# ghostshell202/FluidFramework

Measured on AMD Instinct MI355X. Metric: sequenced ops applied/sec (whole node) over 100k docs, bit-exact summaries, higher is better.
Workload: dtype int32

## Files before the change

### fluidframework_amd/csrc/apply.hip.h

```cpp
#pragma once
#include <hip/hip_runtime.h>
#include <stdint.h>

#include <type_traits>

#include "../../include/mtr_synth.h"
#include "../../include/mtr_types.h"

#define MTR_DI __device__ __forceinline__
#ifndef MTR_COLD_NOINLINE
#define MTR_COLD_NOINLINE 0
#endif
#if MTR_COLD_NOINLINE
#define MTR_COLD __device__ __attribute__((noinline))
#else
#define MTR_COLD MTR_DI
#endif
#ifndef MTR_UNSWITCH
#define MTR_UNSWITCH 1
#endif

namespace mtr {

constexpr int NT = 64;
// ... 122 lines not shown
    uint32_t* heap;
    uint16_t* text;
    uint32_t* prop;
    uint32_t* rm;
    int32_t segcap, hcap, tcap, pcap, rcap;
    int32_t rtab;
    int32_t cap;
    int32_t lhcap;
    int32_t global_mode;
    uint32_t* scratch;
    int32_t ops_this_launch;
    int32_t new_length_calc;
    uint32_t n_docs;
    const uint32_t* doc_list;
    uint32_t n_launch;
    const mtr_op* ops;
    const mtr_doc_desc* docs;
    const uint16_t* btext;
    const uint32_t* propop_off;
    const uint32_t* propop_kv;
    const uint32_t* key_index;
    const uint32_t* val_eq;
    unsigned long long* stat_ops;
    uint32_t* delta;
    const uint64_t* doff;
    const uint32_t* dkind;
    const uint32_t* dpart;
    int32_t gen;
    int32_t gen_grow;
    mtr_synth_cfg gen_cfg;
    mtr_synth_state* gen_state;
    mtr_op* gen_ops;
    uint16_t* gen_text;
    unsigned long long* prof;
    uint32_t* pend;
    int32_t* csum;
    int32_t* umap;
    uint32_t* refs;
    int32_t refcap;
};

enum { P_OP = 0, P_PREFIX, P_SPLIT, P_SHIFT, P_INSERT, P_RANGE, P_ZAMBONI, P_ZBLOCK, P_COMPACT, P_FINDUID,
       P_TEXTGC, P_LOADSTORE, P_TEXTCOPY, P_UPDSEQ, P_NZBLOCK, P_NCOMPACT, P_SCOUR1, P_PACK, P_NLQ, P_PMATCH,
       P_TAPPEND, P_HEAP, P_OVERFLOW, P_NPACK, P_NMERGE, P_NPMATCH, P_NNLQ, P_SPLIT1, P_INS1, P_FETCH, P_X1, P_X2,
       P_PFSUM, P_PFDIRTY, P_MAT, P_CSUM, P_NCH, P_NLISTED, P_NDIRTY,
       P_SPREAD, P_CHUNKOF, P_NSPREAD,
       P_LOAD, P_PRE, P_VIEW, P_POST,
       P_NSUP, P_NDCH,
       P_HELPER,
       P_SINK,
       P_OVB, P_OVPB, P_NOVFB, P_NOVL,
       P_SUPREF, P_PXLIST, P_PXEVAL, P_PXSYNC, P_NPXR,
       P_NWALK, P_NDRND, P_WALK,
       P_COUNT };

enum { CP_TEXT = 0, CP_PROP, CP_RM, CP_RT, CP_DELTA, CP_POFF, CP_PKV, CP_KIX, CP_VEQ, CP_HDR, CP_PEND, CP_CSUM, CP_UMAP,
       CP_REFS, CP_N };

struct Sc {
    unsigned long long cp[CP_N];
    int gen_ref, gen_client;
    int rel[2];
    int relmask;
    int nrefs, refcap;
    int fail_op, max_heap, heap_need;
    int sepoch;
    int vref;
    unsigned long long sum_s, sum_l;
#ifdef MTR_PROF
    unsigned long long prof[P_COUNT];
#endif
};

struct St {
    int nseg, height, minseq, curseq;
    int collab, local, heapn, uidnext;
    int textused, propused, rmused, status;
    int texthalf;
    int htop;
    int dused;
    int holes;
    int chunked;
    int cur_op;
};

struct View {
    int ref;
    uint32_t client;
    int local;
};

template <bool G>
struct Doc {
    template <class T>
    using A = typename std::conditional<G, gptr<T>, lptr<T>>::type;
    A<int> len, seq, rseq, E, hseq;
    A<uint32_t> meta, text, props, uid, huid;
    lptr<Sc> sc;
    lptr<mtr_synth_state> gst;
    lptr<int> sx;
    int dcap;
    int cap, lhcap, rtmask;
    MTR_DI unsigned long long cold(int k) const {
        const unsigned long long v = sc->cp[k];
        return (unsigned long long)(uint32_t)__builtin_amdgcn_readfirstlane(int(uint32_t(v))) |
               ((unsigned long long)(uint32_t)__builtin_amdgcn_readfirstlane(int(uint32_t(v >> 32))) << 32);
    }
// ... 246 lines not shown
                         (newlen ? vp_lt(minseq, rseq) : vis);
        int inr = first;
        if (__ballot(walk != 0)) {
#ifdef MTR_PROF
            PROF_COUNT(P_NWALK);
            ProfScope _prof_walk(L.sc, P_WALK);
#endif
            const int iw = slotp ? (walk != 0 ? *slotp : 0) : i;
            inr |= -later_remover(L, iw, walk != 0, v.client);
        }
        if (newlen) {
            const int live = vis & len;
            const int gone = live & ~(~after | inr);
            return vp_sel(rem, vp_le(rseq, minseq) | gone, live);
        }
        const int seen = len & ~(rem & inr);
        const int r = vp_sel(vis, seen, rem & (X ? vp_lt(rseq, LOCAL_BASE) : -1));
        return r | (rem & ~after);
    }
    static MTR_DI int later_remover(const D& L, int i, bool walk, uint32_t c) {
        int inr = 0;
        if (walk) {
            uint32_t cell = rm_get(L, L.uid[i]);
            while (cell != 0xffffffu) {
                const uint32_t w = L.grm()[cell];
                if ((w >> 24) == c) {
                    inr = 1;
                    break;
                }
                cell = w & 0xffffffu;
            }
        }
        return inr;
    }

    static MTR_DI int local_length(const D& L, const St& s) {
        int sum = 0;
        for (int base = 0; base < s.nseg; base += 64) {
            const int i = base + lane_id();
            int x = 0;
            if (i < s.nseg && L.rseq[i] == RNONE) x = L.len[i];
            sum += rdlane(wave_incl_scan(x), 63);
        }
        return sum;
    }

    static constexpr int EMASK = 0x7fffffff;
    static MTR_DI int ev(int e, int eprev) { return e < 0 ? -1 : e - (eprev & EMASK); }
#ifndef MTR_GK
#define MTR_GK 4
#endif
    static constexpr int GK = MTR_GK;

    static MTR_DI void prefix(D& L, const St& s, const View& v, int newlen) {
        PROF(P_PREFIX);
        const int S = s.nseg;
        const int ln = lane_id();
        int carry = 0;
        if constexpr (G) {
            for (int base = 0; base < S; base += 64 * GK) {
                Hot hk[GK];
#pragma unroll
                for (int q = 0; q < GK; q++) hk[q] = ld_hot(L, min(base + 64 * q + ln, S - 1));
#pragma unroll
                for (int q = 0; q < GK; q++) {
                    if (base + 64 * q >= S) break;
                    const int i = base + 64 * q + ln;
                    const int x0 = vis_hot(L, hk[q], i, v, newlen, s.minseq, i < S);
                    const int in = vp_lt(i, S);
                    const int x = x0 & in;
                    const int inc = wave_incl_scan(max(x, 0));
                    L.E[vp_sel(in, i, S)] = (carry + inc) | (x & int(0x80000000u));
                    carry += rdlane(inc, 63);
                }
            }
            wsync();
            return;
        }
        if (MTR_UNSWITCH && !v.local && !newlen) prefix_lds<0, 0>(L, s, v, 0);
        else prefix_lds<-1, -1>(L, s, v, newlen);
        wsync();
    }
    template <int LOC, int NL>
    static MTR_DI void prefix_lds(D& L, const St& s, const View& v, int newlen) {
        const int S = s.nseg;
        const int ln = lane_id();
        int carry = 0;
        Hot h = S > 0 ? ld_hot(L, ln) : Hot{};
        for (int base = 0; base < S; base += 64) {
            const int i = base + ln;
            const Hot cur = h;
            if (base + 64 < S) h = ld_hot(L, i + 64);
            const int x0 = vis_hot<LOC, NL>(L, cur, i, v, newlen, s.minseq, i < S);
            const int in = vp_lt(i, S);
            const int x = x0 & in;
            const int inc = wave_incl_scan(max(x, 0));
            L.E[vp_sel(in, i, S)] = (carry + inc) | (x & int(0x80000000u));
            carry += rdlane(inc, 63);
        }
    }

    static MTR_DI int nsup(const D& L) { return sup_rows(L.cap); }
    static MTR_DI int nchr(const D& L) { return L.cap / 64 + 1; }
    static MTR_DI gptr<int> cs_rec(const D& L, int c) { return L.gcsum() + c * kCsumRows; }
    static MTR_DI gptr<int> cs_sl(const D& L) { return L.gcsum() + kCsumRows * nchr(L); }
    static MTR_DI gptr<int> cs_se(const D& L) { return cs_sl(L) + nsup(L); }
    static MTR_DI lptr<int> sup_pre(const D& L) { return L.sx; }
    static MTR_DI lptr<int> sup_fill(const D& L) { return L.sx + nsup(L); }
    static MTR_DI lptr<int> sup_mark(const D& L) { return L.sx + 2 * nsup(L); }
    static MTR_DI lptr<int> sup_len(const D& L) { return L.sx + 3 * nsup(L); }
    static MTR_DI lptr<int> sup_ev(const D& L) { return L.sx + 4 * nsup(L); }
    static MTR_DI lptr<int> sup_dlen(const D& L) { return L.sx + 5 * nsup(L); }
    static MTR_DI lptr<int> dlist(const D& L) { return L.sx + 6 * nsup(L); }
    static MTR_DI lptr<int> ch_ev(const D& L) { return dlist(L) + kListCap; }
    static MTR_DI lptr<int> ch_x(const D& L) { return ch_ev(L) + nchr(L); }
    static MTR_DI v4i ld4(gptr<const int> p) { return *(gptr<const v4i>)p; }
    static MTR_DI void csum_update(D& L, const St& s, int lo, int hi) {
        PROF(P_CSUM);
        if constexpr (G) {
            if (!s.chunked) return;
            hi = min(hi, s.nseg);
            if (lo >= hi) return;
            const int c0 = max(lo, 0) >> 6, c1 = (hi - 1) >> 6;
            for (int cb = c0; cb <= c1; cb += GK) {
                uint32_t mq[GK];
                int lq[GK], sqq[GK], rq[GK];
#pragma unroll
                for (int g = 0; g < GK; g++) {
                    const int ic = min((cb + g) * 64 + lane_id(), s.nseg - 1);
                    mq[g] = L.meta[ic];
                    lq[g] = L.len[ic];
                    sqq[g] = L.seq[ic];
                    rq[g] = L.rseq[ic];
                }
#pragma unroll
                for (int g = 0; g < GK; g++) {
                    const int c = cb + g;
                    if (c > c1) break;
                    const int i = c * 64 + lane_id();
                    const bool in = i < s.nseg;
                    const uint32_t m = mq[g];
                    const int len = lq[g], sq = sqq[g], rs = rq[g];
                    const bool live = in && !(m & M_DEL);
                    const bool rem = rs != RNONE;
                    const bool win = live && (sq > s.minseq || (rem && rs > s.minseq));
                    const uint64_t wm = __ballot(win);
                    const int nw = __popcll(wm);
                    int x = (live && !rem) ? len : 0;
                    int fx = (live && !rem && !win) ? len : 0;
                    int ev = live ? max(sq, rem ? rs : 0) : 0;
                    x = rdlane(wave_incl_scan(x), 63);
                    fx = rdlane(wave_incl_scan(fx), 63);
// ... 423 lines not shown
        const int x = ch_ev(L)[cc] > vref ? ch_x(L)[cc] : cl;
        const int inc = wave_incl_scan(c < nch ? x : 0);
        if (c < nch) ch_x(L)[c] = inc;
        if (lane_id() == 0) sup_fill(L)[q] = ep;
        wsync();
        return inc;
    }
    static MTR_DI void materialize(D& L, const St& s, const View& v, int newlen, int c0, int c1) {
        PROF(P_MAT);
        const int S = s.nseg, ln = lane_id();
        const lptr<int> spre = sup_pre(L);
        int qcur = -1, rel = 0;
        for (int cb = c0; cb <= c1; cb += GK) {
            Hot h[GK];
#pragma unroll
            for (int k = 0; k < GK; k++) h[k] = ld_hot(L, min(min(cb + k, c1) * 64 + ln, S - 1));
#pragma unroll
            for (int k = 0; k < GK; k++) {
                const int c = cb + k;
                if (c > c1) break;
                const int q = c >> 6;
                if (q != qcur && (c & 63)) {
                    rel = sup_row(L, s, q);
                    qcur = q;
                }
                const int base = (q > 0 ? uni(spre[q - 1]) : 0) + ((c & 63) ? rdlane(rel, (c & 63) - 1) : 0);
                const int i = c * 64 + ln;
                const int x0 = vis_hot(L, h[k], i, v, newlen, s.minseq, i < S);
                const int x = i < S ? x0 : 0;
                const int inc = wave_incl_scan(max(x, 0));
                if (i < S) L.E[i] = (base + inc) | (x < 0 ? int(0x80000000u) : 0);
            }
        }
        wsync();
    }
    static MTR_DI int chunk_of(D& L, const St& s, int nch, int pos) {
        PROF(P_CHUNKOF);
        const int ns = (nch + 63) >> 6, ln = lane_id();
        const lptr<int> spre = sup_pre(L);
        int q = -1;
        for (int b = 0; b < ns; b += 64) {
            const uint64_t m = __ballot(b + ln < ns && spre[min(b + ln, ns - 1)] >= pos);
            if (m) {
                q = b + first_lane(m);
                break;
            }
        }
        if (q < 0) return nch - 1;
        const int rel = sup_row(L, s, q);
        const int base = q > 0 ? uni(spre[q - 1]) : 0;
        const uint64_t m = __ballot(q * 64 + ln < nch && base + rel >= pos);
        return m ? q * 64 + first_lane(m) : nch - 1;
    }
    static MTR_DI int view_scan(D& L, St& s, const View& v, int newlen, int p_lo, int p_hi, bool bounded = false) {
        PROF(P_VIEW);
        if constexpr (G) {
            L.rhi = 0;
            if (s.chunked && s.nseg > 0) {
                const int total = prefix2(L, s, v, newlen, bounded ? p_hi + 1 : INT32_MAX);
                const int nch = (s.nseg + 63) >> 6;
                const int c0 = max(0, chunk_of(L, s, nch, p_lo) - 1);
                const int c1 = min(nch - 1, chunk_of(L, s, nch, p_hi + 1) + 2);
                materialize(L, s, v, newlen, c0, c1);
                L.rlo = c0 * 64;
                L.rhi = (c1 + 1) * 64;
                return total;
            }
        }
        prefix(L, s, v, newlen);
        return s.nseg > 0 ? (uni(L.E[s.nseg - 1]) & EMASK) : 0;
    }

    static MTR_DI void find1(const D& L, const St& s, const View& v, int pos, int& i_out, int& before, int newlen) {
        const int S = s.nseg;
        const int ln = lane_id();
        int c = 0;
        i_out = S;
        before = 0;
        for (int base = 0; base < S; base += 64) {
            const int i = base + ln;
            const Hot h = ld_hot(L, min(i, S - 1));
            const int x0 = vis_hot(L, h, i, v, newlen, s.minseq, i < S);
            const int x = (i < S) ? max(x0, 0) : 0;
            const int inc = wave_incl_scan(x);
            const uint64_t m = __ballot((i < S) & (c + inc > pos));
            if (m) {
                const int l = first_lane(m);
                i_out = base + l;
                before = c + rdlane(inc - x, l);
                return;
            }
            c += rdlane(inc, 63);
        }
        before = c;
    }

    static MTR_DI void containing(char* smem, const KParams& P, uint32_t d, int pos, int ref, int client, int32_t* out) {
        D L;
        carve(L, smem, P, d);
        St s;
        load_doc(L, P, s, d);
        View v;
        v.ref = ref;
        v.client = enc_client(client);
        v.local = (!s.collab || uint32_t(s.local) == v.client) ? 1 : 0;
        int i, before;
        find1(L, s, v, pos, i, before, P.new_length_calc);
        const int li = (G && s.holes && i < s.nseg) ? count_live(L, 0, i) : i;
        if (lane_id() == 0) {
            if (i >= s.nseg || pos < 0) {
                out[0] = -1;
                out[9] = before;
            } else {
                const uint32_t m = L.meta[i];
                out[0] = li;
                out[1] = pos - before;
                out[2] = L.len[i];
                out[3] = L.seq[i];
                out[4] = dec_client(m & M_CLIENT_MASK);
                out[5] = L.rseq[i] == RNONE ? -1 : L.rseq[i];
                out[6] = (m & M_MARKER) ? 1 : 0;
                out[7] = int(L.text[i]);
// ... 2419 lines not shown
#pragma unroll
            for (int q = 0; q < ZK; q++) {
                const int i = wb + 64 * q + ln;
                const bool it = i < hi && !(mq[q] & M_DEL) && (l == 2 || bnd_of(mq[q]) >= l - 2);
                const uint64_t mask = __ballot(it);
                const int k = n + __popcll(mask & lanes_below());
                if (it && k < 64) lst[k] = i;
                n += __popcll(mask);
            }
        }
        int T = n, off = 0;
        if (W > 1) {
            const lptr<int> row = tbox(L) + 16;
            if (ln == 0) row[w] = n;
            __syncthreads();
            T = 0;
            for (int u = 0; u < W; u++) {
                const int nu = uni(row[u]);
                if (u < w) off += nu;
                T += nu;
                if (nu > 64) T = -(1 << 20);
            }
        } else if (n > 64) {
            T = -1;
        }
        if (T < 0) return -1;
        if (T == 0) return 0;
        const int c = max(1, min(kMaxNodesInBlock - 1, T / (kMaxNodesInBlock / 2)));
        const int base = T / c;
        const int rem = T % c;
        const int big = rem * (base + 1);
        wsync();
        if (ln < n) {
            const int i = lst[ln];
            uint32_t m = L.meta[i];
            const int item = off + ln;
            const bool isStart = item < big ? item % (base + 1) == 0 : (item - big) % base == 0;
            const int nb = item == 0 ? top : (isStart ? l - 1 : (l == 2 ? 0 : l - 2));
            m = set_bnd(m, nb);
            if (l == 2 && isStart) m = set_ns(m, NS_UNDEF);
            L.meta[i] = m;
        }
        wsync();
        return c;
    }

    static MTR_DI int zamboni_block(D& L, const KParams& P, St& s, int x, int& to) {
        PROF(P_ZBLOCK);
        PROF_COUNT(P_NZBLOCK);
        const int H = s.height;
        int rs1, re1;
        block_bounds1(L, s, x, rs1, re1);
        const uint32_t m1 = uniu(L.meta[rs1]);
        if (ns_of(m1) == NS_FALSE) return -1;
        const int topb1 = bnd_of(m1);
        const int before = G && s.holes ? count_live(L, rs1, re1) : re1 - rs1;
        to = re1;
        int kept;
        {
            PROF(P_SCOUR1);
            kept = re1 - rs1 <= 64 ? scour_par(L, P, s, rs1, re1) : scour_gather(L, P, s, rs1, re1);
            if (kept < 0) kept = scour_range(L, P, s, rs1, re1);
        }
        for (int b = rs1; b < re1; b += 64) {
            const int i = b + lane_id();
            const uint64_t m = __ballot(i < re1 && !(L.meta[min(i, re1 - 1)] & M_DEL));
            if (m) {
                const int first = b + first_lane(m);
                L.meta[first] = set_ns(set_bnd(uniu(L.meta[first]), topb1), NS_FALSE);
                wsync();
                break;
            }
        }
        if (kept >= before) return -1;
        int from = rs1;
        if (kept < kMaxNodesInBlock / 2 && H > 1) {
            PROF(P_PACK);
            PROF_COUNT(P_NPACK);
            int cs = rs1, ce = re1;
            for (int l = 2; l <= H; l++) {
                int ps, pe;
                {
                    PROF(P_FETCH);
                    if (G && team_n() > 1) {
                        int cnt;
                        team_bounds(L, s, cs, ce, l, ps, pe, cnt);
                    } else {
                        ps = block_start(L, cs, l);
                        pe = block_end(L, s, ce - 1, l);
                    }
                }
                const int top = bnd_of(uniu(L.meta[ps]));
                cs = ps;
                ce = pe;
                if (l == 2) {
                    from = ps;
                    to = max(to, pe);
                    PROF(P_SPLIT1);
                    if ((pe - ps <= 64 ? scour_par(L, P, s, ps, pe) : scour_gather(L, P, s, ps, pe)) < 0)
                        scour_range(L, P, s, ps, pe);
                }
                {
                    int c = -1;
                    if (G && team_n() > 1) {
                        const lptr<int> b = tbox(L);
                        if (lane_id() == 0) {
                            b[1] = ps;
// ... 26 lines not shown
                    if (wb == ps) m1r = mq[0];
#pragma unroll
                    for (int q = 0; q < ZK; q++)
                        T += __popcll(__ballot(!(mq[q] & M_DEL) && (l == 2 || bnd_of(mq[q]) >= l - 2)));
                }
                int c = 0;
                if (T > 0) {
                    c = min(kMaxNodesInBlock - 1, T / (kMaxNodesInBlock / 2));
                    if (c < 1) c = 1;
                    const int base = T / c;
                    const int rem = T % c;
                    const int big = rem * (base + 1);
                    int item0 = 0;
                    for (int wb = ps; wb < pe; wb += 64 * ZK) {
                        uint32_t mq[ZK];
#pragma unroll
                        for (int q = 0; q < ZK; q++) {
                            const int i = wb + 64 * q + lane_id();
                            mq[q] = pe - ps <= 64 ? m1r : L.meta[min(i, pe - 1)];
                            if (i >= pe) mq[q] = M_DEL;
                        }
#pragma unroll
                        for (int q = 0; q < ZK; q++) {
                            const int i = wb + 64 * q + lane_id();
                            uint32_t m = mq[q];
                            const bool it = !(m & M_DEL) && (l == 2 || bnd_of(m) >= l - 2);
                            const uint64_t mask = __ballot(it);
                            if (it) {
                                const int item = item0 + __popcll(mask & lanes_below());
                                const bool isStart = item < big ? item % (base + 1) == 0 : (item - big) % base == 0;
                                const int nb = item == 0 ? top : (isStart ? l - 1 : (l == 2 ? 0 : l - 2));
                                m = set_bnd(m, nb);
                                if (l == 2 && isStart) m = set_ns(m, NS_UNDEF);
                                L.meta[i] = m;
                            }
                            item0 += __popcll(mask);
                        }
                    }
                    wsync();
                }
                if (!(c < kMaxNodesInBlock / 2 && l < H)) break;
            }
        }
        return from;
    }

    static MTR_DI void zamboni(D& L, const KParams& P, St& s) {
        PROF(P_ZAMBONI);
        if (!s.collab) return;
        for (int it = 0; it < 2; it++) {
            if (s.heapn == 0 || s.status != MTR_OK) return;
            if (s.htop > s.minseq) return;
            const uint32_t u = heap_pop(L, s);
            const int x = find_uid(L, s, u);
            if (x < 0) continue;
            int to = 0;
            const int from = zamboni_block(L, P, s, x, to);
            if (from >= 0) {
                if (G && s.holes) {
                    holeify(L, s, from, to);
                    csum_update(L, s, from, to);
                } else {
                    compact(L, s, from);
                    s.chunked = 0;
                }
            }
        }
    }

    static MTR_DI int update_seq(St& s, int msn, int seq) {
        int run = 0;
        if (s.curseq > seq) {
            s.status = MTR_ERR_ASSERT | 0x038;
        } else {
            s.curseq = seq;
            if (msn > seq) s.status = MTR_ERR_ASSERT | 0x039;
            else if (msn > s.curseq) s.status = MTR_ERR_ASSERT | 0x04e;
            else if (s.minseq > msn) s.status = MTR_ERR_ASSERT | 0x04f;
            else if (msn > s.minseq) {
                s.minseq = msn;
                run = 1;
            }
        }
        return run;
    }

    static MTR_DI void split_at(D& L, const KParams& P, St& s, int pos) {
        PROF(P_SPLIT);
        const int S = s.nseg;
        const int i = lower_bound_E(L, s, pos);
        if (i >= S) return;
        const int ln = lane_id();
        const int jj = i + ln;
        const bool in = jj < S;
        const int jc = min(jj, S - 1);
        const int ej0 = L.E[jc], ep = L.E[max(jc - 1, 0)];
        const uint32_t mj = L.meta[jc], tj = L.text[jc], pj = pget(L, jc), uj = L.uid[jc];
        const int lj = L.len[jc], sqj = L.seq[jc], rsj = L.rseq[jc];
        const int vj = ev(ej0, jc > 0 ? ep : 0);
        const int ej = ej0 & EMASK;
        const uint64_t em = __ballot(!in | (bnd_of(mj) >= 1)) & ~uint64_t(1);
        const int be = em ? i + first_lane(em) : block_end(L, s, i + 63, 1);
        const uint64_t cm = __ballot((jj < be) & (vj >= 0) & (pos < ej));
        if (!cm) return;
        const int jl = first_lane(cm);
        const int j = i + jl;
        const int v = rdlane(vj, jl), e = rdlane(ej, jl);
        const uint32_t m0 = rdlane(mj, jl);
        const int off = pos - (e - v);
        if (!(off > 0 && !(m0 & M_MARKER))) return;
        const bool grew = shift_right1(L, s, j + 1);
        {
            const int r = j + 1;
            L.len[r] = rdlane(lj, jl) - off;
            L.len[j] = off;
            L.seq[r] = rdlane(sqj, jl);
            L.rseq[r] = rdlane(rsj, jl);
            L.meta[r] = set_ns(set_bnd(m0, 0), NS_UNDEF);
            L.meta[j] = (m0 & M_NONL) ? (m0 & ~M_NL) : ((m0 & ~M_NL) | M_NLQ);
            {
                const uint32_t t0 = rdlane(tj, jl);
                L.text[r] = t0 == uint32_t(MTR_HANDLE_UNALLOCATED) ? t0 : t0 + uint32_t(off);
            }
            pset(L, r, (PM && rdlane(pj, jl) != NONE32) ? track_split(L, P, s, rdlane(pj, jl)) : rdlane(pj, jl));
            const uint32_t ur = uint32_t(s.uidnext++);
            L.uid[r] = ur;
            if (G && s.chunked && lane_id() == 0) hint(L, ur, r);
            if constexpr (X) {
                if (nrefs(L)) {
                    wsync();
                    ref_split(L, uniu(rdlane(uj, jl)), off, ur);
                }
            }
            if (m0 & M_OVERLAP) {
                if (lane_id() == 0 && !rm_set(L, ur, rm_get(L, rdlane(uj, jl)))) s.status = MTR_ERR_CAPACITY;
                s.status = uni(s.status);
            }
            L.E[j] = e - v + off;
            L.E[r] = e;
            wsync();
            if (X && (m0 & (M_PEND | M_ZOMB))) pend_copy(L, P, s, uniu(rdlane(uj, jl)), r);
            if (grew) s.nseg++;
            if (G) csum_update(L, s, j, max(L.shi, r + 1));
            overflow_fix(L, s, r);
        }
    }

    static MTR_DI int insert_at(D& L, const KParams& P, St& s, const View& v, const mtr_op& op, int pos, int seq,
                                uint32_t client, const mtr_doc_desc& dd, bool pre, uint32_t pf, int sseq, int lseq,
                                int force = -1) {
        PROF(P_INSERT);
        const bool marker = (op.flags & MTR_F_MARKER) != 0;
        const int len = marker ? 1 : int(op.payload2);
        if (len <= 0) return -1;
        const int t0 = s.textused;
        const int ln = lane_id();
        if (!marker && !PM) {
            if (t0 + len > text_end(s, P)) {
                s.status = MTR_ERR_CAPACITY;
                return -1;
            }
            PROF(P_TEXTCOPY);
        }
        bool nl = false, nonl = false;
        if (!marker && !PM) {
            bool any = false, last = false;
            if (pre) {
                if (ln < len) {
                    L.gtext()[t0 + ln] = uint16_t(pf);
                    any = pf == u'\n';
                    last = any && ln == len - 1;
                }
            } else {
                const gptr<const uint16_t> src = gp(P.btext) + dd.text_base + op.payload;
                for (int k = ln; k < len; k += 64) {
                    const uint16_t u = src[k];
                    L.gtext()[t0 + k] = u;
                    if (u == u'\n') {
                        any = true;
                        last = last || k == len - 1;
                    }
                }
            }
            nonl = __ballot(any) == 0;
            nl = __ballot(last) != 0;
        }
        const int S = s.nseg;
        int slot = -1, inherit = 0;
        bool nocand = false;
        uint32_t om = 0;
        bool om_known = false;
        int wbs = -1, wbe = -1;
        if (force >= 0) {
            slot = force;
            inherit = slot == block_start(L, slot, 1) ? 1 : 0;
        } else {
            PROF(P_INS1);
            if (S == 0) {
                if (pos == 0) slot = 0;
                else s.status = MTR_ERR_INSERT_FAILED;
            } else {
                const int i = lower_bound_E(L, s, pos);
                if (i >= S) {
                    s.status = MTR_ERR_INSERT_FAILED;
                } else {
                    const int w = i - 31 + ln;
                    const bool inw = (w >= 0) & (w < S);
                    const int wc = min(max(w, 0), S - 1);
                    const int ew0 = L.E[wc], ewp = L.E[max(wc - 1, 0)], sw = L.seq[wc];
                    const uint32_t mw = L.meta[wc];
                    const int vw = ev(ew0, wc > 0 ? ewp : 0);
                    const int ew = ew0 & EMASK;
                    const bool bw = inw & (bnd_of(mw) >= 1);
                    const uint64_t sm = __ballot((w <= 0) | bw) & LO32;
                    const uint64_t em = __ballot((w >= S) | bw) & HI32;
#ifdef MTR_DEBUG_INSERT
                    {
                        const uint32_t mw2 = __atomic_load_n((uint32_t*)&L.meta[wc], __ATOMIC_RELAXED);
                        const uint64_t b1 = __ballot(bw), b2 = __ballot(inw & (bnd_of(mw2) >= 1));
                        const uint64_t dm = __ballot(mw != mw2);
                        if (b1 != b2 && lane_id() == 0)
                            printf("MISMATCH op_begin %llu i %d ballot(bw) %llx fresh %llx meta-differs %llx\n",
                                   (unsigned long long)dd.op_begin, i, (unsigned long long)b1, (unsigned long long)b2,
                                   (unsigned long long)dm);
                    }
#endif
                    if (sm && em) {
                        const int bs = max(0, i - 31 + last_lane(sm));
                        const int be = i - 31 + first_lane(em);
                        const uint64_t cm = (HI32 | (uint64_t(1) << 31)) & __ballot((w < be) & (vw >= 0) &
                                                     ((ew > pos) | ((vw == 0) & (seq > sw))));
                        slot = cm ? i - 31 + first_lane(cm) : be;
                        nocand = !cm;
                        inherit = slot == bs ? 1 : 0;
                        wbs = bs;
                        wbe = be + 1;
                        if (inherit) {
                            om = uint32_t(rdlane(int(mw), bs - i + 31));
                            om_known = true;
                        }
                    } else {
                        const int bs = block_start(L, i, 1), be = block_end(L, s, i, 1);
                        slot = be;
                        nocand = true;
                        for (int jb = i; jb < be; jb += 64) {
                            const int j = jb + ln;
                            bool c = false;
                            if (j < be) {
                                const int ej = L.E[j];
                                const int vj = ev(ej, j > 0 ? L.E[j - 1] : 0);
                                c = vj >= 0 && ((ej & EMASK) > pos || (vj == 0 && seq > L.seq[j]));
                            }
                            const uint64_t cm = __ballot(c);
                            if (cm) {
                                slot = jb + first_lane(cm);
// ... 163 lines not shown
                               gptr<const uint16_t> btext) {
        PROF(P_LOAD);
        const int ln = lane_id();
        const uint32_t ty = ow[0] & 0xffu, fl = (ow[0] >> 8) & 0xffu;
        const bool el = ln >= t0 && ln < tend && ty == MTR_OP_LOAD &&
                        !(fl & (MTR_F_MARKER | MTR_F_PROPS | MTR_F_REL)) && int(ow[3]) <= 0;
        const uint64_t bad = __ballot(!el) & ~((uint64_t(1) << t0) - 1);
        const int cnt = (bad ? first_lane(bad) : 64) - t0;
        if (cnt <= 0) return 0;
        const bool act = ln >= t0 && ln < t0 + cnt;
        const int len = act ? int(ow[7]) : 0;
        const int incl = wave_incl_scan(len);
        const int tot = rdlane(incl, 63);
        if (s.nseg + cnt + 3 > L.cap || s.textused + tot + 4096 > text_end(s, P)) return 0;
        if (act) {
            const int i = s.nseg + (ln - t0);
            const uint32_t t = uint32_t(s.textused + incl - len);
            const gptr<const uint16_t> src = btext + ow[6];
            for (int q = 0; q < len; q++) L.gtext()[t + q] = src[q];
            L.len[i] = len;
            L.seq[i] = int(ow[1]);
            L.rseq[i] = int(ow[2]) >= 0 ? int(ow[2]) : RNONE;
            L.meta[i] = enc_client(int(int16_t(ow[0] >> 16))) | M_NLQ | ((fl & MTR_F_NOREF) ? M_NOREF : 0u);
            L.text[i] = t;
            pset(L, i, NONE32);
            L.uid[i] = uint32_t(s.uidnext + (ln - t0));
        }
        wsync();
        s.nseg += cnt;
        s.uidnext += cnt;
        s.textused += tot;
        return cnt;
    }

    static MTR_COLD void finish_load(D& L, St& s) {
        PROF(P_LOAD);
        const int S = s.nseg;
        int H = 1;
        for (int n = S; n > kMaxNodesInBlock - 1; n = (n + kMaxNodesInBlock - 2) / (kMaxNodesInBlock - 1)) H++;
        for (int i = lane_id(); i < S; i += 64) {
            int b = 0;
            if (i == 0) {
                b = H;
            } else {
                for (int64_t p = kMaxNodesInBlock - 1; b + 1 < H && i % p == 0; p *= kMaxNodesInBlock - 1) b++;
            }
            L.meta[i] = set_ns(set_bnd(L.meta[i], b), NS_UNDEF);
        }
        wsync();
        s.height = H;
        if (G && !PM && S >= kGapMin) spread(L, s, L.cap);
    }

    static MTR_DI void range_walk(D& L, const KParams& P, St& s, const View& v, int start, int end, int seq,
                                  uint32_t client, int is_remove, uint32_t pp, uint32_t comb, bool dl,
                                  bool pending = false, int plseq = 0) {
        PROF(P_RANGE);
        if (end == start) return;
        const int S = s.nseg;
        const int ln = lane_id();
        const bool lru = s.collab && !v.local;
        int last_blk = -1;
        int pslot = -1;
        L.wlo = lower_bound_E(L, s, start + 1);
        L.whi = L.wlo;
        for (int base = L.wlo; base < S; base += 64) {
            L.whi = min(base + 64, S);
            const int j = base + ln;
            const bool in = j < S;
            const int jc = min(j, S - 1);
            const int ej0 = L.E[jc], ep = L.E[max(jc - 1, 0)], rj = L.rseq[jc];
            uint32_t mj = L.meta[jc];
            const int vj = ev(ej0, jc > 0 ? ep : 0);
            const int ej = ej0 & EMASK;
            const uint64_t stop = __ballot(!in | (ej - max(vj, 0) >= end));
            const int lim = stop ? first_lane(stop) : 64;
            const bool act = (ln < lim) & (vj > 0);
            const uint64_t am = __ballot(act);
            if (am) {
                if (is_remove) {
                    const int rs = act ? rj : RNONE;
                    const bool pr = X && act && rs != RNONE && rs >= LOCAL_BASE;
                    const bool ov = act && rs != RNONE && !pr;
                    const uint64_t om = __ballot(ov | pr);
                    const int nov = __popcll(om);
                    if (s.rmused + nov > P.rcap) {
                        s.status = MTR_ERR_CAPACITY;
                        return;
                    }
                    bool full = false;
                    if (ov) {
                        const uint32_t cell = uint32_t(s.rmused + __popcll(om & lanes_below()));
                        const uint32_t uj = L.uid[j];
                        const uint32_t nxt = (mj & M_OVERLAP) ? rm_get(L, uj) : 0xffffffu;
                        L.grm()[cell] = (client << 24) | (nxt & 0xffffffu);
                        full = !rm_set(L, uj, cell);
                        mj |= M_OVERLAP;
                        L.meta[j] = mj;
                    } else if (pr) {
                        const uint32_t cell = uint32_t(s.rmused + __popcll(om & lanes_below()));
                        const uint32_t uj = L.uid[j];
                        L.grm()[cell] = (((mj >> M_FREM_SHIFT) & 0xffu) << 24) | 0xffffffu;
                        uint32_t t = (mj & M_OVERLAP) ? rm_get(L, uj) : 0xffffffu;
                        if (t == 0xffffffu) {
                            full = !rm_set(L, uj, cell);
                        } else {
                            while ((L.grm()[t] & 0xffffffu) != 0xffffffu) t = L.grm()[t] & 0xffffffu;
                            L.grm()[t] = (L.grm()[t] & 0xff000000u) | cell;
                        }
                        L.rseq[j] = seq;
                        mj = (mj & ~(0xffu << M_FREM_SHIFT)) | (client << M_FREM_SHIFT) | M_OVERLAP;
                        L.meta[j] = mj;
                    } else if (act) {
                        L.rseq[j] = seq;
                        mj = (mj & ~(0xffu << M_FREM_SHIFT) & ~M_OVERLAP) | (client << M_FREM_SHIFT);
                        if (dl) mj |= M_TOUCH;
                        L.meta[j] = mj;
// ... 408 lines not shown
            wsync();
        }
        if (op.type == MTR_OP_LOAD) {
            PROF(P_LOAD);
            load_leaf(L, P, s, op, dd);
            if (s.status != MTR_OK) {
                set_fail(L, gidx);
                return false;
            }
            return true;
        }
        if (s.height == 0) finish_load(L, s);
        if (G && !PM && s.nseg >= kGapMin &&
            (s.holes * 64 < s.nseg || (s.holes && s.nseg + 2 >= L.cap) || s.holes > 3 * (s.nseg - s.holes)))
            spread(L, s, L.cap);
        const bool local_op = op.type >= MTR_OP_LOCAL_INSERT && op.type <= MTR_OP_LOCAL_ANNOTATE;
        int zop = 0;
        View v;
        int seq = op.seq;
        int sseq = 0, lseq = 0;
        uint32_t client = enc_client(int(int16_t(op.client)));
        if (local_op) {
            v.ref = s.curseq;
            v.local = 1;
            if (s.collab) {
                if (!X) {
                    s.status = MTR_ERR_UNSUPPORTED;
                    set_fail(L, gidx);
                    return false;
                }
                lseq = uni(L.ghdr()->lseq) + 1;
                if (lane_id() == 0) L.ghdr()->lseq = lseq;
                v.client = uint32_t(s.local);
                client = uint32_t(s.local);
                seq = TIE_LOCAL;
                sseq = LOCAL_BASE + lseq;
            } else {
                v.client = CL_LOCAL;
                seq = 0;
                client = CL_LOCAL;
            }
        } else {
            v.ref = (op.flags & MTR_F_APPEND) ? 0 : op.ref_seq;
            v.client = client;
            v.local = (!s.collab || uint32_t(s.local) == client) ? 1 : 0;
        }
        PROF_ADD(P_PRE, _t_pre);
        if (X && op.type == MTR_OP_RELPOS) view_scan(L, s, v, P.new_length_calc, 0, 0);
        switch (op.type) {
            case MTR_OP_INSERT:
            case MTR_OP_LOCAL_INSERT: {
                int pos = pos1;
                if (op.flags & MTR_F_APPEND) pos = local_length(L, s);
                view_scan(L, s, v, P.new_length_calc, pos, pos, true);
                int force = -1;
                if (PM && local_op && op.pos2 >= 0) {
                    force = track_ref_slot(L, P, s, uint32_t(op.pos2));
                    if (force < 0) {
                        s.status = MTR_ERR_BAD_OP;
                        break;
                    }
                } else {
                    split_at(L, P, s, pos);
                }
                const int at = insert_at(L, P, s, v, op, pos, seq, client, dd, pre, pf, lseq ? sseq : seq, lseq, force);
                if (PM && local_op && at >= 0 && s.status == MTR_OK) {
                    if (op.payload) track_link(L, P, s, at, op.payload);
                    if (op.pos2 >= 0 && s.status == MTR_OK) {
                        if (!op.payload) s.status = MTR_ERR_BAD_OP;
                        else track_transfer(L, P, s, at, uint32_t(op.pos2));
                    }
                }
                zop = s.collab && !local_op;
                break;
            }
            case MTR_OP_REMOVE:
            case MTR_OP_LOCAL_REMOVE:
            case MTR_OP_ANNOTATE:
            case MTR_OP_LOCAL_ANNOTATE: {
                const int is_remove = op.type == MTR_OP_REMOVE || op.type == MTR_OP_LOCAL_REMOVE;
                view_scan(L, s, v, P.new_length_calc, min(pos1, pos2), max(pos1, pos2), true);
                split_at(L, P, s, pos1);
                split_at(L, P, s, pos2);
                const bool track = PM && op.type == MTR_OP_LOCAL_REMOVE && op.payload != 0;
                if (X && lseq) {
                    range_walk(L, P, s, v, pos1, pos2, sseq, client, is_remove, op.payload, is_remove ? 0u : op.payload2,
                               is_remove != 0, true, lseq);
                    if (track && s.status == MTR_OK) track_touched(L, P, s, op.payload, false);
                    if (s.status == MTR_OK && is_remove) pend_touched(L, P, s, PK_REMOVE, 0u, lseq);
                } else {
                    range_walk(L, P, s, v, pos1, pos2, seq, client, is_remove, op.payload,
                               (op.type == MTR_OP_ANNOTATE || (X && op.type == MTR_OP_LOCAL_ANNOTATE)) ? op.payload2 : 0u,
                               (DL && !PM && (op.flags & MTR_F_DELTA) != 0) || track);
                    if (track && s.status == MTR_OK) track_touched(L, P, s, op.payload, true);
                }
                if (X && is_remove && !lseq && s.status == MTR_OK && nrefs(L)) ref_slide_walk(L, s, seq);
                if (G && is_remove) csum_update(L, s, L.wlo, L.whi);
                zop = s.collab && !local_op;
                break;
            }
            case MTR_OP_SEQ:
                break;
            case MTR_OP_ROLLBACK:
                if (!X || !s.collab) {
                    s.status = MTR_ERR_BAD_OP;
                    break;
                }
                rollback(L, P, s, int(op.payload2), op.payload, uint32_t(op.pos1));
                break;
            case MTR_OP_REGENERATE:
                if (!X || !DL || !s.collab) {
                    s.status = MTR_ERR_BAD_OP;
                    break;
                }
                regenerate(L, P, s, int(op.payload2), gidx);
                break;
            case MTR_OP_ACK:
                if (!X || !s.collab) {
                    s.status = MTR_ERR_BAD_OP;
                    break;
                }
                ack(L, s, int(op.payload2), op.seq);
                zop = 1;
                break;
            case MTR_OP_HANDLES: {
                const int n = op.pos1;
                if (!X || !PM || s.collab || n < 1) {
                    s.status = MTR_ERR_BAD_OP;
                } else if (n > handle_cap(P)) {
                    s.status = MTR_ERR_CAPACITY;
                } else {
                    load_handles(gp(P.btext) + dd.text_base + op.payload, handles(L), n);
                    s.textused = n;
                    wsync();
                }
                break;
            }
            case MTR_OP_RELPOS: {
                const uint64_t mu = X ? mk_look(L.grt(), uint32_t(L.rtmask), uint32_t(op.pos1)) : 0;
                int p = -1;
                if (mu >> 32) {
                    const int x = find_uid(L, s, uint32_t(mu));
                    if (G && L.rhi > 0 && x > 0) materialize(L, s, v, P.new_length_calc, (x - 1) >> 6, (x - 1) >> 6);
                    p = x > 0 ? (uni(L.E[x - 1]) & EMASK) : 0;
                    const int off = (op.payload2 & MTR_REL_OFFSET) ? int(op.payload) : 0;
                    p = (op.payload2 & MTR_REL_BEFORE) ? p - off : p + 1 + off;
// ... 500 lines not shown
```

### fluidframework_amd/engine.py

```python
from __future__ import annotations

import ctypes as C
import os

import numpy as np

from . import abi, gitid

_HERE = os.path.dirname(os.path.abspath(__file__))
_LIB = None


class EngineError(RuntimeError):
    pass


class MtrCaps(C.Structure):
    _fields_ = [
        ("max_segments", C.c_uint32),
        ("heap_entries", C.c_uint32),
        ("text_units", C.c_uint32),
        ("prop_words", C.c_uint32),
        ("remover_cells", C.c_uint32),
        ("ops_per_launch", C.c_uint32),
# ... 732 lines not shown
    def export(self, doc):
        h = C.c_int32(0)
        n = lib().mtr_export(self.h, doc, None, 0, C.byref(h))
        n = -n if n < 0 else n
        out = np.zeros((max(n, 1), 8), dtype="<i4")
        lib().mtr_export(self.h, doc, out.ctypes.data, n, C.byref(h))
        return out[:n], h.value

    def stats(self) -> dict:
        out = np.zeros(10, dtype="<i8")
        self._check(lib().mtr_stats(self.h, out.ctypes.data, 10), "mtr_stats")
        keys = ["ops", "docs", "max_leaves", "sum_leaves", "bad_docs", "launches", "max_heap", "max_text",
                "sum_leaves_before_op", "text_units_inserted"]
        return dict(zip(keys, (int(x) for x in out)))

    def profile(self, reset=True) -> dict:
        out = np.zeros(len(PROFILE_KEYS), dtype="<u8")
        if lib().mtr_profile(self.h, out.ctypes.data, len(PROFILE_KEYS), int(reset)) != 0:
            return {}
        return dict(zip(PROFILE_KEYS, (int(x) for x in out)))

    def launch_counts(self) -> dict:
        tail = ["fixed_cap", "min_cap", "max_cap", "global_mode", "max_lds_cap"]
        n = len(LAUNCH_VARIANTS) + len(tail)
        out = np.zeros(n, dtype="<i8")
        got = lib().mtr_debug_launch_counts(self.h, out.ctypes.data, n)
        if got != n:
            raise EngineError(f"mtr_debug_launch_counts: the library reports {got} counters, this binding knows {n}")
        res = dict(zip(LAUNCH_VARIANTS + tail, (int(x) for x in out)))
        res["launches"] = sum(res[k] for k in LAUNCH_VARIANTS) + res["fixed_cap"]
        return res

    def timing(self) -> dict:
        out = np.zeros(17, dtype="<f8")
        lib().mtr_last_timing(self.h, out.ctypes.data, 17)
        return {"apply_ms": float(out[0]), "summary_ms": float(out[1]), "apply_launches": int(out[2]),
                "apply_kernel_ms": float(out[3]), "blob_ids_ms": float(out[4]), "delta_ms": float(out[5]),
                "delta_gather_ms": float(out[6]), "tree_ids_ms": float(out[7]), "novel_ms": float(out[8]),
                "novel_gather_ms": float(out[9]), "novel_classify_ms": float(out[10]),
                "cache_trim_ms": float(out[11]), "cache_ages_ms": float(out[12]),
                "handover_copied_bytes": float(out[13]), "handover_ids_ms": float(out[14]),
                "handover_novel_ms": float(out[15]), "handover_ranges": int(out[16])}


LAUNCH_VARIANTS = ["LDS_X", "HBM_X", "LDS_LEAN", "HBM_LEAN", "LDS_DL", "HBM_DL", "LDS_GN", "HBM_GN", "PAIR_LDS",
                   "PAIR_HBM", "PAIR_LDS_DL", "PAIR_HBM_DL", "PAIR_LDS_GN", "PAIR_HBM_GN", "PAIR2_LDS", "PAIR2_HBM"]

PROFILE_KEYS = ["op", "prefix", "split", "shift", "insert", "range", "zamboni", "zblock", "compact", "find_uid",
                "text_gc", "loadstore", "text_copy", "update_seq", "n_zblock", "n_compact", "scour1", "pack", "nlq",
                "pmatch", "tappend", "heap", "overflow", "n_pack", "n_merge", "n_pmatch", "n_nlq", "split1", "ins1",
                "fetch", "x1", "x2", "pf_sum", "pf_dirty", "materialize", "csum", "n_chunks", "n_listed", "n_dirty", "spread", "chunk_of", "n_spread",
                "load", "pre", "view", "post", "n_sup", "n_dch", "helper", "sink",
                "ovf_bounds", "ovf_parent", "n_ovf_nowin", "n_ovf_rounds", "sup_refresh", "px_list_eval", "px_eval",
                "px_sync", "n_px_rounds", "n_walk", "n_dirty_rounds", "walk"]


def caps_for(batch, margin=1.25):
    ops = batch.ops
    docs = batch.docs
    n_ops = docs["op_count"].astype(np.int64)
    max_ops = int(n_ops.max()) if len(docs) else 0
    max_text = int(docs["text_count"].max()) if len(docs) else 0
    seg = 2 * max_ops + 64
    text = int(2 * max_text * margin) + 4096
    npk = np.diff(batch.propop_off.astype(np.int64)) if len(batch.propop_off) > 1 else np.zeros(1, np.int64)
    max_keys = int(npk.max()) if npk.size else 0
    prop = int((2 * max_ops) * (1 + 2 * (max_keys + 8)) * 0.25) + 4096
    rem = max_ops + 64
    return dict(max_segments=seg, heap_entries=seg, text_units=text, prop_words=prop, remover_cells=rem)
```

Measured before the change: 429.3 million.

## Derive split/insert/range positions from prefix scan ballots instead of binary searches

The LDS prefix scan now counts, via wave ballots, how many segments have prefix below or at the requested positions. Insert, split and range-walk use these counts in place of separate lower_bound_E searches. split_at also looks back 31 lanes so it can find the block start and pass tighter bounds to overflow_fix. In exchange the scan does extra ballots per 64-segment chunk, the index must be adjusted after the first split, and correctness depends on that adjustment. Profiling counters for heap pops are also added.

```diff
diff --git a/fluidframework_amd/csrc/apply.hip.h b/fluidframework_amd/csrc/apply.hip.h
--- a/fluidframework_amd/csrc/apply.hip.h
+++ b/fluidframework_amd/csrc/apply.hip.h
@@ -198,7 +198,9 @@
        P_OVB, P_OVPB, P_NOVFB, P_NOVL,
        P_SUPREF, P_PXLIST, P_PXEVAL, P_PXSYNC, P_NPXR,
        P_NWALK, P_NDRND, P_WALK,
+       P_NPOP, P_NPOPNOOP,
        P_COUNT };
+static_assert(P_COUNT <= 64, "mtr_profile reads 64 slots");
 
 enum { CP_TEXT = 0, CP_PROP, CP_RM, CP_RT, CP_DELTA, CP_POFF, CP_PKV, CP_KIX, CP_VEQ, CP_HDR, CP_PEND, CP_CSUM, CP_UMAP,
        CP_REFS, CP_N };
@@ -551,7 +553,11 @@
 #endif
     static constexpr int GK = MTR_GK;
 
-    static MTR_DI void prefix(D& L, const St& s, const View& v, int newlen) {
+    struct Hits {
+        int lo = -1, hi = -1, lo1 = -1;
+    };
+    static MTR_DI void prefix(D& L, const St& s, const View& v, int newlen, int p_lo = 0, int p_hi = 0,
+                              Hits* hits = nullptr) {
         PROF(P_PREFIX);
         const int S = s.nseg;
         const int ln = lane_id();
@@ -576,15 +582,18 @@
             wsync();
             return;
         }
-        if (MTR_UNSWITCH && !v.local && !newlen) prefix_lds<0, 0>(L, s, v, 0);
-        else prefix_lds<-1, -1>(L, s, v, newlen);
+        Hits h;
+        if (MTR_UNSWITCH && !v.local && !newlen) prefix_lds<0, 0>(L, s, v, 0, p_lo, p_hi, h);
+        else prefix_lds<-1, -1>(L, s, v, newlen, p_lo, p_hi, h);
+        if (hits) *hits = h;
         wsync();
     }
     template <int LOC, int NL>
-    static MTR_DI void prefix_lds(D& L, const St& s, const View& v, int newlen) {
+    static MTR_DI void prefix_lds(D& L, const St& s, const View& v, int newlen, int p_lo, int p_hi, Hits& hits) {
         const int S = s.nseg;
         const int ln = lane_id();
         int carry = 0;
+        int n_lo = 0, n_hi = 0, n_lo1 = 0;
         Hot h = S > 0 ? ld_hot(L, ln) : Hot{};
         for (int base = 0; base < S; base += 64) {
             const int i = base + ln;
@@ -595,8 +604,15 @@
             const int x = x0 & in;
             const int inc = wave_incl_scan(max(x, 0));
             L.E[vp_sel(in, i, S)] = (carry + inc) | (x & int(0x80000000u));
+            const int cq = vp_sel(in, carry + inc, EMASK);
+            n_lo += __popcll(__ballot(cq < p_lo));
+            n_hi += __popcll(__ballot(cq < p_hi));
+            n_lo1 += __popcll(__ballot(cq <= p_lo));
             carry += rdlane(inc, 63);
         }
+        hits.lo = n_lo;
+        hits.hi = n_hi;
+        hits.lo1 = n_lo1;
     }
 
     static MTR_DI int nsup(const D& L) { return sup_rows(L.cap); }
@@ -1126,7 +1142,8 @@
         const uint64_t m = __ballot(q * 64 + ln < nch && base + rel >= pos);
         return m ? q * 64 + first_lane(m) : nch - 1;
     }
-    static MTR_DI int view_scan(D& L, St& s, const View& v, int newlen, int p_lo, int p_hi, bool bounded = false) {
+    static MTR_DI int view_scan(D& L, St& s, const View& v, int newlen, int p_lo, int p_hi, bool bounded = false,
+                                Hits* hits = nullptr) {
         PROF(P_VIEW);
         if constexpr (G) {
             L.rhi = 0;
@@ -1141,7 +1158,7 @@
                 return total;
             }
         }
-        prefix(L, s, v, newlen);
+        prefix(L, s, v, newlen, p_lo, p_hi, G ? nullptr : hits);
         return s.nseg > 0 ? (uni(L.E[s.nseg - 1]) & EMASK) : 0;
     }
 
@@ -3667,7 +3684,10 @@
         int rs1, re1;
         block_bounds1(L, s, x, rs1, re1);
         const uint32_t m1 = uniu(L.meta[rs1]);
-        if (ns_of(m1) == NS_FALSE) return -1;
+        if (ns_of(m1) == NS_FALSE) {
+            PROF_COUNT(P_NPOPNOOP);
+            return -1;
+        }
         const int topb1 = bnd_of(m1);
         const int before = G && s.holes ? count_live(L, rs1, re1) : re1 - rs1;
         to = re1;
@@ -3800,8 +3820,12 @@
             if (s.heapn == 0 || s.status != MTR_OK) return;
             if (s.htop > s.minseq) return;
             const uint32_t u = heap_pop(L, s);
+            PROF_COUNT(P_NPOP);
             const int x = find_uid(L, s, u);
-            if (x < 0) continue;
+            if (x < 0) {
+                PROF_COUNT(P_NPOPNOOP);
+                continue;
+            }
             int to = 0;
             const int from = zamboni_block(L, P, s, x, to);
             if (from >= 0) {
@@ -3833,30 +3857,39 @@
         return run;
     }
 
-    static MTR_DI void split_at(D& L, const KParams& P, St& s, int pos) {
+    template <bool H = false>
+    static MTR_DI bool split_at(D& L, const KParams& P, St& s, int pos, int hit = -1) {
         PROF(P_SPLIT);
         const int S = s.nseg;
-        const int i = lower_bound_E(L, s, pos);
-        if (i >= S) return;
+        const int i = (H && !G) ? hit : lower_bound_E(L, s, pos);
+        if (i >= S) return false;
+        constexpr int BACK = G ? 0 : 31;
         const int ln = lane_id();
-        const int jj = i + ln;
-        const bool in = jj < S;
-        const int jc = min(jj, S - 1);
+        const int jj = i - BACK + ln;
+        const bool in = (jj >= 0) & (jj < S);
+        const int jc = min(max(jj, 0), S - 1);
         const int ej0 = L.E[jc], ep = L.E[max(jc - 1, 0)];
         const uint32_t mj = L.meta[jc], tj = L.text[jc], pj = pget(L, jc), uj = L.uid[jc];
         const int lj = L.len[jc], sqj = L.seq[jc], rsj = L.rseq[jc];
         const int vj = ev(ej0, jc > 0 ? ep : 0);
         const int ej = ej0 & EMASK;
-        const uint64_t em = __ballot(!in | (bnd_of(mj) >= 1)) & ~uint64_t(1);
-        const int be = em ? i + first_lane(em) : block_end(L, s, i + 63, 1);
-        const uint64_t cm = __ballot((jj < be) & (vj >= 0) & (pos < ej));
-        if (!cm) return;
+        const bool bj = in & (bnd_of(mj) >= 1);
+        constexpr uint64_t UPTO = (uint64_t(2) << BACK) - 1;
+        const uint64_t em = __ballot((jj >= S) | bj) & ~UPTO;
+        const int be = em ? i - BACK + first_lane(em) : block_end(L, s, i - BACK + 63, 1);
+        int bs = -1;
+        if constexpr (!G) {
+            const uint64_t sm = __ballot((jj <= 0) | bj) & UPTO;
+            bs = sm ? max(0, i - BACK + last_lane(sm)) : block_start(L, i, 1);
+        }
+        const uint64_t cm = __ballot((jj < be) & (vj >= 0) & (pos < ej)) & ~(UPTO >> 1);
+        if (!cm) return false;
         const int jl = first_lane(cm);
-        const int j = i + jl;
+        const int j = i - BACK + jl;
         const int v = rdlane(vj, jl), e = rdlane(ej, jl);
         const uint32_t m0 = rdlane(mj, jl);
         const int off = pos - (e - v);
-        if (!(off > 0 && !(m0 & M_MARKER))) return;
+        if (!(off > 0 && !(m0 & M_MARKER))) return false;
         const bool grew = shift_right1(L, s, j + 1);
         {
             const int r = j + 1;
@@ -3890,13 +3923,16 @@
             if (X && (m0 & (M_PEND | M_ZOMB))) pend_copy(L, P, s, uniu(rdlane(uj, jl)), r);
             if (grew) s.nseg++;
             if (G) csum_update(L, s, j, max(L.shi, r + 1));
-            overflow_fix(L, s, r);
-        }
-    }
-
+            if constexpr (G) overflow_fix(L, s, r);
+            else overflow_fix(L, s, r, bs, be + 1);
+        }
+        return true;
+    }
+
+    template <bool H = false>
     static MTR_DI int insert_at(D& L, const KParams& P, St& s, const View& v, const mtr_op& op, int pos, int seq,
                                 uint32_t client, const mtr_doc_desc& dd, bool pre, uint32_t pf, int sseq, int lseq,
-                                int force = -1) {
+                                int force = -1, int hit = -1) {
         PROF(P_INSERT);
         const bool marker = (op.flags & MTR_F_MARKER) != 0;
         const int len = marker ? 1 : int(op.payload2);
@@ -3948,7 +3984,7 @@
                 if (pos == 0) slot = 0;
                 else s.status = MTR_ERR_INSERT_FAILED;
             } else {
-                const int i = lower_bound_E(L, s, pos);
+                const int i = (H && !G) ? hit : lower_bound_E(L, s, pos);
                 if (i >= S) {
                     s.status = MTR_ERR_INSERT_FAILED;
                 } else {
@@ -4218,9 +4254,10 @@
         if (G && !PM && S >= kGapMin) spread(L, s, L.cap);
     }
 
+    template <bool H = false>
     static MTR_DI void range_walk(D& L, const KParams& P, St& s, const View& v, int start, int end, int seq,
                                   uint32_t client, int is_remove, uint32_t pp, uint32_t comb, bool dl,
-                                  bool pending = false, int plseq = 0) {
+                                  bool pending = false, int plseq = 0, int hit = -1) {
         PROF(P_RANGE);
         if (end == start) return;
         const int S = s.nseg;
@@ -4228,7 +4265,7 @@
         const bool lru = s.collab && !v.local;
         int last_blk = -1;
         int pslot = -1;
-        L.wlo = lower_bound_E(L, s, start + 1);
+        L.wlo = (H && !G) ? hit : lower_bound_E(L, s, start + 1);
         L.whi = L.wlo;
         for (int base = L.wlo; base < S; base += 64) {
             L.whi = min(base + 64, S);
@@ -4743,7 +4780,8 @@
             case MTR_OP_LOCAL_INSERT: {
                 int pos = pos1;
                 if (op.flags & MTR_F_APPEND) pos = local_length(L, s);
-                view_scan(L, s, v, P.new_length_calc, pos, pos, true);
+                Hits hit;
+                view_scan(L, s, v, P.new_length_calc, pos, pos, true, &hit);
                 int force = -1;
                 if (PM && local_op && op.pos2 >= 0) {
                     force = track_ref_slot(L, P, s, uint32_t(op.pos2));
@@ -4752,9 +4790,10 @@
                         break;
                     }
                 } else {
-                    split_at(L, P, s, pos);
-                }
-                const int at = insert_at(L, P, s, v, op, pos, seq, client, dd, pre, pf, lseq ? sseq : seq, lseq, force);
+                    split_at<true>(L, P, s, pos, hit.lo);
+                }
+                const int at = insert_at<true>(L, P, s, v, op, pos, seq, client, dd, pre, pf, lseq ? sseq : seq, lseq,
+                                               force, hit.lo);
                 if (PM && local_op && at >= 0 && s.status == MTR_OK) {
                     if (op.payload) track_link(L, P, s, at, op.payload);
                     if (op.pos2 >= 0 && s.status == MTR_OK) {
@@ -4770,19 +4809,26 @@
             case MTR_OP_ANNOTATE:
             case MTR_OP_LOCAL_ANNOTATE: {
                 const int is_remove = op.type == MTR_OP_REMOVE || op.type == MTR_OP_LOCAL_REMOVE;
-                view_scan(L, s, v, P.new_length_calc, min(pos1, pos2), max(pos1, pos2), true);
-                split_at(L, P, s, pos1);
-                split_at(L, P, s, pos2);
+                Hits hit;
+                view_scan(L, s, v, P.new_length_calc, min(pos1, pos2), max(pos1, pos2), true, &hit);
+                const bool fwd = pos1 <= pos2;
+                int i1 = hit.lo, i2 = hit.hi, wlo = hit.lo1;
+                if (!G && !fwd) i1 = lower_bound_E(L, s, pos1);
+                const int up = split_at<true>(L, P, s, pos1, i1) ? 1 : 0;
+                if (!G) i2 = fwd ? i2 + (pos2 > pos1 ? up : 0) : lower_bound_E(L, s, pos2);
+                split_at<true>(L, P, s, pos2, i2);
+                if (!G) wlo = fwd ? wlo + up : lower_bound_E(L, s, pos1 + 1);
                 const bool track = PM && op.type == MTR_OP_LOCAL_REMOVE && op.payload != 0;
                 if (X && lseq) {
-                    range_walk(L, P, s, v, pos1, pos2, sseq, client, is_remove, op.payload, is_remove ? 0u : op.payload2,
-                               is_remove != 0, true, lseq);
+                    range_walk<true>(L, P, s, v, pos1, pos2, sseq, client, is_remove, op.payload,
+                                     is_remove ? 0u : op.payload2, is_remove != 0, true, lseq, wlo);
                     if (track && s.status == MTR_OK) track_touched(L, P, s, op.payload, false);
                     if (s.status == MTR_OK && is_remove) pend_touched(L, P, s, PK_REMOVE, 0u, lseq);
                 } else {
-                    range_walk(L, P, s, v, pos1, pos2, seq, client, is_remove, op.payload,
-                               (op.type == MTR_OP_ANNOTATE || (X && op.type == MTR_OP_LOCAL_ANNOTATE)) ? op.payload2 : 0u,
-                               (DL && !PM && (op.flags & MTR_F_DELTA) != 0) || track);
+                    range_walk<true>(L, P, s, v, pos1, pos2, seq, client, is_remove, op.payload,
+                                     (op.type == MTR_OP_ANNOTATE || (X && op.type == MTR_OP_LOCAL_ANNOTATE)) ? op.payload2
+                                                                                                            : 0u,
+                                     (DL && !PM && (op.flags & MTR_F_DELTA) != 0) || track, false, 0, wlo);
                     if (track && s.status == MTR_OK) track_touched(L, P, s, op.payload, true);
                 }
                 if (X && is_remove && !lseq && s.status == MTR_OK && nrefs(L)) ref_slide_walk(L, s, seq);
diff --git a/fluidframework_amd/engine.py b/fluidframework_amd/engine.py
--- a/fluidframework_amd/engine.py
+++ b/fluidframework_amd/engine.py
@@ -808,7 +808,7 @@
                 "fetch", "x1", "x2", "pf_sum", "pf_dirty", "materialize", "csum", "n_chunks", "n_listed", "n_dirty", "spread", "chunk_of", "n_spread",
                 "load", "pre", "view", "post", "n_sup", "n_dch", "helper", "sink",
                 "ovf_bounds", "ovf_parent", "n_ovf_nowin", "n_ovf_rounds", "sup_refresh", "px_list_eval", "px_eval",
-                "px_sync", "n_px_rounds", "n_walk", "n_dirty_rounds", "walk"]
+                "px_sync", "n_px_rounds", "n_walk", "n_dirty_rounds", "walk", "n_pop", "n_pop_noop"]
 
 
 def caps_for(batch, margin=1.25):
```

Result: faster. 441.5 million (median of 6 runs) (+2.8%).
